# Nahuel-M/StereoVisionArray

Measured on NVIDIA B200. Metric: MDE/s, higher is better.
Workload: dtype u16

## Files before the change

stereovisionarray_b200/csrc/k_box.cu:

```cuda
#include <algorithm>

#include "sva_common.cuh"

#define BOX_THREADS 256
#define BOX_DP 16
#define BOX_CG 16
#define BOX_MAX_BAND 512

struct BoxParams {
    const uint16_t* A;
    void* out;
    int W, H, D, k, dmin, shift, cap;
    int gxp, gxn, gyp, gyn;
    int band_rows, txo;
    int apply_validity;
};

__device__ __forceinline__ int axis_limit(int pos, int dim, int k, int gp, int gn) {
    if (pos < k || pos >= dim - k) return -1;
    int lim = 0x7FFFFFFF;
    if (gp > 0) lim = min(lim, (pos - k) / gp);
    if (gn > 0) lim = min(lim, (dim - k - pos) / gn);
    return lim;
}

#define BOX_STAGES 3

__device__ __forceinline__ void box_cp16(uint32_t dst, const void* src, int src_bytes) {
    asm volatile("cp.async.cg.shared.global [%0], [%1], 16, %2;" ::"r"(dst), "l"(src), "r"(src_bytes) : "memory");
}

template <int NC, bool RAW>
__global__ void __launch_bounds__(BOX_THREADS, NC == 8 ? 3 : 4)
k_box_cost(BoxParams q) {
    constexpr int TXI = BOX_CG * NC;
    constexpr int ROW_BYTES = TXI * 64;
    constexpr int STAGE_BYTES = 2 * ROW_BYTES;
    extern __shared__ __align__(16) unsigned char box_smem[];
    unsigned char* s_ring = box_smem;
    uint2 (*s_P)[BOX_DP] = reinterpret_cast<uint2 (*)[BOX_DP]>(box_smem + BOX_STAGES * STAGE_BYTES);
    uint2 (*s_tot)[BOX_DP] = reinterpret_cast<uint2 (*)[BOX_DP]>(box_smem + BOX_STAGES * STAGE_BYTES + TXI * BOX_DP * 8);
    int* s_limy = reinterpret_cast<int*>(box_smem + BOX_STAGES * STAGE_BYTES + TXI * BOX_DP * 8 + BOX_CG * BOX_DP * 8);

    const int t = threadIdx.x, dp = t & (BOX_DP - 1), cg = t >> 4;
    const int W = q.W, H = q.H, D = q.D, k = q.k;
    const int d0 = blockIdx.y * 32;
    const int d = d0 + 2 * dp;
    const bool d_ok = d < D;
    const int xs = blockIdx.x * q.txo - k;
    const int y0 = blockIdx.z * q.band_rows, y1 = min(H, y0 + q.band_rows);
    if (y0 >= H) return;

    for (int i = t; i < y1 - y0; i += BOX_THREADS) s_limy[i] = q.apply_validity ? axis_limit(y0 + i, H, k, q.gyp, q.gyn) : 0x7FFFFFFF;

    int limx[NC];
    uint32_t v0[NC], v1[NC];
#pragma unroll
    for (int j = 0; j < NC; j++) {
        int x = xs + cg * NC + j;
        limx[j] = q.apply_validity ? axis_limit(x, W, k, q.gxp, q.gxn) : 0x7FFFFFFF;
        v0[j] = 0; v1[j] = 0;
    }
    const long long rowstride = (long long)W * D;
    const uint32_t ring_base = (uint32_t)__cvta_generic_to_shared(s_ring);

    auto fill = [&](int it) {
        const uint32_t st = ring_base + ((it + 2 * k) % BOX_STAGES) * STAGE_BYTES;
        const int ra = y0 + it + k - 1, rs = y0 + it - k;
        const bool ra_ok = ra >= 0 && ra < H, rs_ok = it >= 0 && rs >= 0 && rs < H;
#pragma unroll
        for (int c = t; c < TXI * 4; c += BOX_THREADS) {
            const int col = c >> 2, part = c & 3, x = xs + col, dd = d0 + 8 * part;
            const bool in = x >= 0 && x < W && dd < D;
            const long long off = ((long long)(in ? x : 0)) * D + (in ? dd : 0);
            box_cp16(st + c * 16, q.A + (ra_ok ? ra : 0) * rowstride + off, (in && ra_ok) ? 16 : 0);
            if (it >= 0) box_cp16(st + ROW_BYTES + c * 16, q.A + (rs_ok ? rs : 0) * rowstride + off, (in && rs_ok) ? 16 : 0);
        }
    };

    const int it_begin = -(2 * k - 1), it_end = y1 - y0;
#pragma unroll
    for (int i = 0; i < BOX_STAGES - 1; i++) {
        if (it_begin + i < it_end) fill(it_begin + i);
        asm volatile("cp.async.commit_group;" ::: "memory");
    }

    for (int it = it_begin; it < it_end; it++) {
        asm volatile("cp.async.wait_group %0;" ::"n"(BOX_STAGES - 2) : "memory");
        __syncthreads();
        if (it + BOX_STAGES - 1 < it_end) fill(it + BOX_STAGES - 1);
        asm volatile("cp.async.commit_group;" ::: "memory");
        const unsigned char* st = s_ring + ((it + 2 * k) % BOX_STAGES) * STAGE_BYTES;
        const uint32_t* rowa = reinterpret_cast<const uint32_t*>(st) + (cg * NC) * 16 + dp;
#pragma unroll
        for (int j = 0; j < NC; j++) { uint32_t w = rowa[j * 16]; v0[j] += w & 0xFFFFu; v1[j] += w >> 16; }
        if (it < 0) continue;
        const int y = y0 + it;
        uint32_t p0[NC], p1[NC];
        uint32_t a0 = 0, a1 = 0;
#pragma unroll
        for (int j = 0; j < NC; j++) { a0 += v0[j]; a1 += v1[j]; p0[j] = a0; p1[j] = a1; }
        s_tot[cg][dp] = make_uint2(a0, a1);
        __syncthreads();
        uint32_t o0 = 0, o1 = 0;
        for (int g = 0; g < cg; g++) { uint2 tt = s_tot[g][dp]; o0 += tt.x; o1 += tt.y; }
#pragma unroll
        for (int j = 0; j < NC; j++) s_P[cg * NC + j][dp] = make_uint2(p0[j] + o0, p1[j] + o1);
        __syncthreads();
        const int limy = s_limy[it];
#pragma unroll
        for (int j = 0; j < NC; j++) {
            int ci = cg * NC + j, x = xs + ci;
            if (ci < k || ci > TXI - k || x >= W || ci - k >= q.txo || !d_ok) continue;
            uint2 hi = s_P[ci + k - 1][dp];
            uint2 lo = (ci - k - 1 >= 0) ? s_P[ci - k - 1][dp] : make_uint2(0u, 0u);
            uint32_t r0 = hi.x - lo.x, r1 = hi.y - lo.y;
            int lim = min(limx[j], limy);
            bool ok0 = q.dmin + d <= lim, ok1 = q.dmin + d + 1 <= lim;
            long long o = ((long long)y * W + x) * D + d;
            if (RAW) {
                *reinterpret_cast<uint2*>((uint32_t*)q.out + o) = make_uint2(ok0 ? r0 : 0xFFFFFFFFu, ok1 ? r1 : 0xFFFFFFFFu);
            } else {
                uint32_t c0 = ok0 ? min((uint32_t)q.cap, r0 >> q.shift) : (uint32_t)q.cap;
                uint32_t c1 = ok1 ? min((uint32_t)q.cap, r1 >> q.shift) : (uint32_t)q.cap;
                *reinterpret_cast<uint32_t*>((uint16_t*)q.out + o) = c0 | (c1 << 16);
            }
        }
        const uint32_t* rows = reinterpret_cast<const uint32_t*>(st + ROW_BYTES) + (cg * NC) * 16 + dp;
#pragma unroll
        for (int j = 0; j < NC; j++) { uint32_t w = rows[j * 16]; v0[j] -= w & 0xFFFFu; v1[j] -= w >> 16; }
    }
}

template <int NC, bool RAW>
static cudaError_t box_launch(const BoxParams& q, dim3 grid, cudaStream_t stream) {
    constexpr int TXI = BOX_CG * NC;
    const size_t smem = (size_t)BOX_STAGES * 2 * TXI * 64 + (size_t)TXI * BOX_DP * 8 + BOX_CG * BOX_DP * 8 + BOX_MAX_BAND * 4;
    cudaError_t e = cudaFuncSetAttribute(k_box_cost<NC, RAW>, cudaFuncAttributeMaxDynamicSharedMemorySize, (int)smem);
    if (e != cudaSuccess) return e;
    k_box_cost<NC, RAW><<<grid, BOX_THREADS, smem, stream>>>(q);
    return cudaGetLastError();
}

int sva_launch_box(sva_ctx* ctx, const uint16_t* A, void* out, int W, int H, int D, int k, const sva_params* prm, bool raw, bool apply_validity) {
    if (k < 1 || k > 56) return ctx->fail(SVA_ERR_BAD_ARG, "win_half must be in 1..56");
    if (D % 8) return ctx->fail(SVA_ERR_BAD_ARG, "box filter needs a multiple of 8 planes");
    BoxParams q{};
    q.A = A; q.out = out; q.W = W; q.H = H; q.D = D; q.k = k;
    q.dmin = prm ? prm->min_disp : 0; q.shift = prm ? prm->cost_shift : 0; q.cap = prm ? prm->cost_cap : SVA_COST_CAP_MAX;
    q.apply_validity = apply_validity ? 1 : 0;
    if (prm && apply_validity) {
        for (int i = 0; i < prm->n_pairs; i++) {
            int gx = prm->pair_gx[i], gy = prm->pair_gy[i];
            if (gx > 0) q.gxp = gx > q.gxp ? gx : q.gxp;
            if (gx < 0) q.gxn = -gx > q.gxn ? -gx : q.gxn;
            if (gy > 0) q.gyp = gy > q.gyp ? gy : q.gyp;
            if (gy < 0) q.gyn = -gy > q.gyn ? -gy : q.gyn;
        }
    }
    const bool wide = k > 12;
    const int txi = wide ? 128 : 64;
    q.txo = txi - 2 * k + 1;
    int strips = div_up(W, q.txo), dch = div_up(D, 32);
    int bands = div_up(2 * ctx->sm_count * 2, strips * dch);
    int min_band = 4 * k > 32 ? 4 * k : 32;
    if (bands > H / min_band) bands = H / min_band;
    if (bands < 1) bands = 1;
    if (div_up(H, bands) > BOX_MAX_BAND) bands = div_up(H, BOX_MAX_BAND);
    q.band_rows = div_up(H, bands);
    bands = div_up(H, q.band_rows);
    dim3 grid(strips, dch, bands);
    LaunchScope ls(ctx, raw ? "k_box_cost_raw" : "k_box_cost");
    cudaError_t e;
    if (wide) e = raw ? box_launch<8, true>(q, grid, ctx->stream) : box_launch<8, false>(q, grid, ctx->stream);
    else e = raw ? box_launch<4, true>(q, grid, ctx->stream) : box_launch<4, false>(q, grid, ctx->stream);
    SVA_CUDA_OK(ctx, e);
    return SVA_OK;
}

#define BXP_WARPS 8
#define BXP_TCOLS 48
#define BXP_OPITCH 260
#define BXP_MAX_BAND 1024

struct BoxPParams {
    const uint32_t* AP;
    uint16_t* C;
    int W, H, D, k, kk, dmin, shift, cap;
    int gxp, gxn, gyp, gyn;
    int band_rows, txo, wp;
    int l2hint;
    int chunk;
    long long row_words;
    int ry0, ry1;
};

__global__ void __launch_bounds__(256, 2)
k_box_planar(BoxPParams q) {
    __shared__ __align__(16) uint32_t s_out[2][BXP_WARPS][BXP_OPITCH];
    __shared__ __align__(8) unsigned long long s_bar[2];
    __shared__ uint2 s_T[BXP_WARPS][8 * BXP_TCOLS];
    __shared__ int s_limy[BXP_MAX_BAND];
    const int t = threadIdx.x, lane = t & 31, warp = t >> 5;
    const int W = q.W, H = q.H, D = q.D, k = q.k;
    const int dpc = min((int)blockIdx.y * BXP_WARPS + warp, (D >> 1) - 1);
    const int d = 2 * dpc;
    const int xs = blockIdx.x * q.txo - q.kk;
    const int y0 = q.ry0 + blockIdx.z * q.band_rows, y1 = min(q.ry1, y0 + q.band_rows);
    for (int i = t; i < y1 - y0; i += 256) s_limy[i] = axis_limit(y0 + i, H, k, q.gyp, q.gyn);

    int thr[8], thrmin = 0x7FFFFFFF;
#pragma unroll
    for (int j = 0; j < 8; j++) {
        thr[j] = axis_limit(xs + lane * 8 + j, W, k, q.gxp, q.gxn) - q.dmin - d;
        thrmin = min(thrmin, thr[j]);
    }
    uint2* tbl = &s_T[warp][8 + lane];
    if (lane == 0) tbl[0] = make_uint2(0u, 0u);
    const uint32_t bar0 = (uint32_t)__cvta_generic_to_shared(&s_bar[0]);
    if (t == 0) {
        asm volatile("mbarrier.init.shared::cta.b64 [%0], %1;" ::"r"(bar0), "r"(BXP_WARPS) : "memory");
        asm volatile("mbarrier.init.shared::cta.b64 [%0], %1;" ::"r"(bar0 + 8), "r"(BXP_WARPS) : "memory");
    }
    int offh[8], offl[8];
#pragma unroll
    for (int j = 0; j < 8; j++) {
        offh[j] = ((j + k) & 7) * BXP_TCOLS + ((j + k) >> 3);
        offl[j] = ((j - k) & 7) * BXP_TCOLS + ((j - k) >> 3);
    }
    __syncthreads();

    const uint32_t* pz = q.AP + (size_t)dpc * q.wp + (size_t)blockIdx.x * q.txo + lane * 8;
    const uint32_t* pe = pz + (size_t)y0 * q.row_words;
    const long long back = 2LL * k * q.row_words;
    const int N = (y1 - y0) + 2 * k - 1;
    uint32_t F[8], Vh[8];
#pragma unroll
    for (int j = 0; j < 8; j++) { F[j] = 0; Vh[j] = 0; }

    const int hf = t & 1;
    const bool half_ok = (int)blockIdx.y * 16 + 8 * hf < D;
    const int xl0 = t >> 1, xl1 = xl0 + 128;
    const bool st0 = half_ok && xl0 >= q.kk && xl0 < q.kk + q.txo && xs + xl0 < W;
    const bool st1 = half_ok && xl1 >= q.kk && xl1 < q.kk + q.txo && xs + xl1 < W;
    uint16_t* po = q.C + ((size_t)y0 * W + (xs + xl0)) * D + blockIdx.y * 16 + 8 * hf;
    const size_t orow = (size_t)W * D;
    const uint32_t kB = (uint32_t)k << 16;

    auto store_row = [&](const int r) {
        const uint32_t bar = bar0 + 8 * (r & 1), parity = (uint32_t)(r >> 1) & 1u;
        asm volatile(
            "{\n"
            ".reg .pred p;\n"
            "BOXWAIT_%=:\n"
            "mbarrier.try_wait.parity.shared::cta.b64 p, [%0], %1;\n"
            "@p bra BOXDONE_%=;\n"
            "bra BOXWAIT_%=;\n"
            "BOXDONE_%=:\n"
            "}" ::"r"(bar), "r"(parity) : "memory");
        const uint32_t* src = &s_out[r & 1][4 * hf][xl0];
        if (st0) *reinterpret_cast<uint4*>(po) = make_uint4(src[0], src[BXP_OPITCH], src[2 * BXP_OPITCH], src[3 * BXP_OPITCH]);
        if (st1) *reinterpret_cast<uint4*>(po + 128 * D) = make_uint4(src[128], src[BXP_OPITCH + 128], src[2 * BXP_OPITCH + 128], src[3 * BXP_OPITCH + 128]);
        po += orow;
    };
    auto row = [&](const int n, const uint4& e0, const uint4& e1, const uint4& l0, const uint4& l1) {
        {
            const uint32_t ee[8] = {e0.x, e0.y, e0.z, e0.w, e1.x, e1.y, e1.z, e1.w};
            const uint32_t ll[8] = {l0.x, l0.y, l0.z, l0.w, l1.x, l1.y, l1.z, l1.w};
#pragma unroll
            for (int j = 0; j < 8; j++) {
                const uint32_t u = ee[j] - ll[j] + 0x80008000u;
                F[j] += u;
                Vh[j] += u >> 16;
            }
        }
        if (n < 2 * k - 1) return;
        const int it = n - (2 * k - 1);
        uint32_t pF[8], pV[8];
        pF[0] = F[0]; pV[0] = Vh[0];
#pragma unroll
        for (int j = 1; j < 8; j++) { pF[j] = pF[j - 1] + F[j]; pV[j] = pV[j - 1] + Vh[j]; }
        uint32_t incF = pF[7], incV = pV[7];
#pragma unroll
        for (int s = 1; s < 32; s <<= 1) {
            const uint32_t a = __shfl_up_sync(0xffffffffu, incF, s), b = __shfl_up_sync(0xffffffffu, incV, s);
            if (lane >= s) { incF += a; incV += b; }
        }
        const uint32_t exF = incF - pF[7], exV = incV - pV[7];
        __syncwarp();
#pragma unroll
        for (int j = 0; j < 8; j++)
            tbl[((j + 1) & 7) * BXP_TCOLS + ((j + 1) >> 3)] = make_uint2(pF[j] + exF, pV[j] + exV);
        __syncwarp();
        const uint32_t B = (uint32_t)(n + 1) * kB, B2 = B * 65537u;
        const int srow = s_limy[it] - q.dmin - d;
        uint32_t w[8];
        if (__all_sync(0xffffffffu, min(thrmin, srow) >= 1)) {
#pragma unroll
            for (int j = 0; j < 8; j++) {
                const uint2 hi = tbl[offh[j]], lo = tbl[offl[j]];
                const uint32_t chi = hi.y - lo.y - B;
                const uint32_t clo = hi.x - lo.x - B2 - (chi << 16);
                const uint32_t c0 = min(clo >> q.shift, (uint32_t)q.cap), c1 = min(chi >> q.shift, (uint32_t)q.cap);
                w[j] = c1 * 65536u + c0;
            }
        } else {
#pragma unroll
            for (int j = 0; j < 8; j++) {
                const uint2 hi = tbl[offh[j]], lo = tbl[offl[j]];
                const uint32_t chi = hi.y - lo.y - B;
                const uint32_t clo = hi.x - lo.x - B2 - (chi << 16);
                uint32_t c0 = min(clo >> q.shift, (uint32_t)q.cap), c1 = min(chi >> q.shift, (uint32_t)q.cap);
                const int m = min(thr[j], srow);
                c0 = m >= 0 ? c0 : (uint32_t)q.cap;
                c1 = m >= 1 ? c1 : (uint32_t)q.cap;
                w[j] = c1 * 65536u + c0;
            }
        }
        if (it > 0) store_row(it - 1);
        uint32_t* so = &s_out[it & 1][warp][lane * 8];
        *reinterpret_cast<uint4*>(so) = make_uint4(w[0], w[1], w[2], w[3]);
        *reinterpret_cast<uint4*>(so + 4) = make_uint4(w[4], w[5], w[6], w[7]);
        __syncwarp();
        if (lane == 0) asm volatile("mbarrier.arrive.shared::cta.b64 _, [%0];" ::"r"(bar0 + 8 * (it & 1)) : "memory");
    };

    uint4 a0 = ldg_stream_u128(pe), a1 = ldg_stream_u128(pe + 4), al0 = make_uint4(0, 0, 0, 0), al1 = al0;
    uint4 b0 = a0, b1 = a1, bl0 = al0, bl1 = al1;
    auto fetch = [&](const int n, uint4& e0, uint4& e1, uint4& l0, uint4& l1) {
        if (n < N) {
            pe += q.row_words;
            const uint32_t* pl = n >= 2 * k ? pe - back : pz;
            e0 = ldg_stream_u128(pe); e1 = ldg_stream_u128(pe + 4);
            l0 = ldg_stream_u128(pl); l1 = ldg_stream_u128(pl + 4);
        }
    };
    for (int n = 0; n < N; n += 2) {
        fetch(n + 1, b0, b1, bl0, bl1);
        row(n, a0, a1, al0, al1);
        if (n + 1 >= N) break;
        fetch(n + 2, a0, a1, al0, al1);
        row(n + 1, b0, b1, bl0, bl1);
    }
    store_row(y1 - y0 - 1);
}

template <int K, int PF, int OCC>
__global__ void __launch_bounds__(256, OCC)
k_box_planar_shfl(BoxPParams q) {
    static_assert(K % 8 == 4 && K >= 4 && K <= 56, "window half-width must be 4 mod 8");
    constexpr int M = (K - 4) / 8;
    __shared__ __align__(16) uint32_t s_out[2][BXP_WARPS][BXP_OPITCH];
    __shared__ __align__(8) unsigned long long s_bar[2];
    __shared__ int s_limy[BXP_MAX_BAND];
    const int t = threadIdx.x, lane = t & 31, warp = t >> 5;
    const int W = q.W, H = q.H, D = q.D;
    const int dpc = min((int)blockIdx.y * BXP_WARPS + warp, (D >> 1) - 1);
    const int d = 2 * dpc;
    const int xs = blockIdx.x * q.txo - K;
    const int y0 = q.ry0 + blockIdx.z * q.band_rows, y1 = min(q.ry1, y0 + q.band_rows);
    for (int i = t; i < y1 - y0; i += 256) s_limy[i] = axis_limit(y0 + i, H, K, q.gyp, q.gyn);

    int thr[8], thrmin = 0x7FFFFFFF;
#pragma unroll
    for (int j = 0; j < 8; j++) {
        thr[j] = axis_limit(xs + lane * 8 + j, W, K, q.gxp, q.gxn) - q.dmin - d;
        thrmin = min(thrmin, thr[j]);
    }
    const uint32_t bar0 = (uint32_t)__cvta_generic_to_shared(&s_bar[0]);
    if (t == 0) {
        asm volatile("mbarrier.init.shared::cta.b64 [%0], %1;" ::"r"(bar0), "r"(BXP_WARPS) : "memory");
        asm volatile("mbarrier.init.shared::cta.b64 [%0], %1;" ::"r"(bar0 + 8), "r"(BXP_WARPS) : "memory");
    }
    __syncthreads();

    const unsigned long long pol_enter = q.l2hint ? l2_policy_evict_last() : l2_policy_evict_normal();
    const unsigned long long pol_leave = q.l2hint ? l2_policy_evict_first() : l2_policy_evict_normal();
    const uint32_t* pe = q.AP + (size_t)dpc * q.wp + (size_t)blockIdx.x * q.txo + lane * 8 + (size_t)y0 * q.row_words;
    const long long back = 2LL * K * q.row_words;
    const int N = (y1 - y0) + 2 * K - 1;
    uint32_t F[8], Hh[8];
#pragma unroll
    for (int j = 0; j < 8; j++) { F[j] = 0; Hh[j] = 0; }

    const int hf = t & 1;
    const bool half_ok = (int)blockIdx.y * 16 + 8 * hf < D;
    const int xl0 = t >> 1, xl1 = xl0 + 128;
    const bool st0 = half_ok && xl0 >= K && xl0 < K + q.txo && xs + xl0 < W;
    const bool st1 = half_ok && xl1 >= K && xl1 < K + q.txo && xs + xl1 < W;
    uint16_t* po = q.C + ((size_t)y0 * W + (xs + xl0)) * D + blockIdx.y * 16 + 8 * hf;
    const size_t orow = (size_t)W * D;

    auto store_row = [&](const int r) {
        const uint32_t bar = bar0 + 8 * (r & 1), parity = (uint32_t)(r >> 1) & 1u;
        asm volatile(
            "{\n"
            ".reg .pred p;\n"
            "BOXSWAIT_%=:\n"
            "mbarrier.try_wait.parity.shared::cta.b64 p, [%0], %1;\n"
            "@p bra BOXSDONE_%=;\n"
            "bra BOXSWAIT_%=;\n"
            "BOXSDONE_%=:\n"
            "}" ::"r"(bar), "r"(parity) : "memory");
        const uint32_t* src = &s_out[r & 1][4 * hf][xl0];
        if (st0) stg_u128_hint(po, make_uint4(src[0], src[BXP_OPITCH], src[2 * BXP_OPITCH], src[3 * BXP_OPITCH]), pol_leave);
        if (st1) stg_u128_hint(po + 128 * D, make_uint4(src[128], src[BXP_OPITCH + 128], src[2 * BXP_OPITCH + 128], src[3 * BXP_OPITCH + 128]), pol_leave);
        po += orow;
    };
    auto hpass = [&](const uint32_t (&u)[8]) {
        uint32_t tF = ((u[0] + u[1]) + (u[2] + u[3])) + ((u[4] + u[5]) + (u[6] + u[7]));
        uint32_t tH = (((u[0] >> 16) + (u[1] >> 16)) + ((u[2] >> 16) + (u[3] >> 16))) + (((u[4] >> 16) + (u[5] >> 16)) + ((u[6] >> 16) + (u[7] >> 16)));
        uint32_t dF[8], dH[8];
        dF[4] = tF; dH[4] = tH;
#pragma unroll
        for (int s = 1; s <= M; s++) {
            dF[4] += __shfl_up_sync(0xffffffffu, tF, s) + __shfl_down_sync(0xffffffffu, tF, s);
            dH[4] += __shfl_up_sync(0xffffffffu, tH, s) + __shfl_down_sync(0xffffffffu, tH, s);
        }
#pragma unroll
        for (int i = 0; i < 3; i++) {
            const uint32_t hi = __shfl_down_sync(0xffffffffu, u[i], M + 1);
            const uint32_t lo = M == 0 ? u[i] : __shfl_up_sync(0xffffffffu, u[i], M == 0 ? 1 : M);
            dF[5 + i] = dF[4 + i] + hi - lo;
            dH[5 + i] = dH[4 + i] + (uint32_t)((int32_t)(hi - lo + 0x8000u) >> 16);
        }
#pragma unroll
        for (int i = 0; i < 4; i++) {
            const uint32_t hi = M == 0 ? u[7 - i] : __shfl_down_sync(0xffffffffu, u[7 - i], M == 0 ? 1 : M);
            const uint32_t lo = __shfl_up_sync(0xffffffffu, u[7 - i], M + 1);
            dF[3 - i] = dF[4 - i] - hi + lo;
            dH[3 - i] = dH[4 - i] - (uint32_t)((int32_t)(hi - lo + 0x8000u) >> 16);
        }
        constexpr uint32_t BF = (uint32_t)(2 * K) * 0x80008000u, BH = (uint32_t)(2 * K) * 0x8000u;
#pragma unroll
        for (int j = 0; j < 8; j++) { F[j] += dF[j] - BF; Hh[j] += dH[j] - BH; }
    };
    auto emit = [&](const int it) {
        const int srow = s_limy[it] - q.dmin - d;
        uint32_t w[8];
        if (__all_sync(0xffffffffu, min(thrmin, srow) >= 1)) {
#pragma unroll
            for (int j = 0; j < 8; j++) {
                const uint32_t chi = Hh[j], clo = F[j] - (chi << 16);
                const uint32_t c0 = min(clo >> q.shift, (uint32_t)q.cap), c1 = min(chi >> q.shift, (uint32_t)q.cap);
                w[j] = c1 * 65536u + c0;
            }
        } else {
#pragma unroll
            for (int j = 0; j < 8; j++) {
                const uint32_t chi = Hh[j], clo = F[j] - (chi << 16);
                uint32_t c0 = min(clo >> q.shift, (uint32_t)q.cap), c1 = min(chi >> q.shift, (uint32_t)q.cap);
                const int m = min(thr[j], srow);
                c0 = m >= 0 ? c0 : (uint32_t)q.cap;
                c1 = m >= 1 ? c1 : (uint32_t)q.cap;
                w[j] = c1 * 65536u + c0;
            }
        }
        if (it > 0) store_row(it - 1);
        uint32_t* so = &s_out[it & 1][warp][lane * 8];
        const bool swz = (lane & 4) != 0;
        *reinterpret_cast<uint4*>(so + (swz ? 4 : 0)) = swz ? make_uint4(w[4], w[5], w[6], w[7]) : make_uint4(w[0], w[1], w[2], w[3]);
        *reinterpret_cast<uint4*>(so + (swz ? 0 : 4)) = swz ? make_uint4(w[0], w[1], w[2], w[3]) : make_uint4(w[4], w[5], w[6], w[7]);
        __syncwarp();
        if (lane == 0) asm volatile("mbarrier.arrive.shared::cta.b64 _, [%0];" ::"r"(bar0 + 8 * (it & 1)) : "memory");
    };

    {
        uint32_t acc[8];
#pragma unroll
        for (int j = 0; j < 8; j++) acc[j] = 0x80008000u;
        int cnt = 0;
        U32x8 a = ldg_stream_u256(pe, pol_enter);
        for (int n = 0; n < 2 * K - 1; n++) {
            U32x8 b = a;
            if (n + 1 < 2 * K - 1) { pe += q.row_words; b = ldg_stream_u256(pe, pol_enter); }
#pragma unroll
            for (int j = 0; j < 8; j++) acc[j] += a.v[j];
            if (++cnt == q.chunk || n + 1 == 2 * K - 1) {
                hpass(acc);
#pragma unroll
                for (int j = 0; j < 8; j++) acc[j] = 0x80008000u;
                cnt = 0;
            }
            a = b;
        }
    }
    {
        const int R = y1 - y0;
        auto fetch = [&](const int it, U32x8& e, U32x8& l) {
            if (it < R) {
                pe += q.row_words;
                e = ldg_stream_u256(pe, pol_enter);
                if (it > 0) l = ldg_stream_u256(pe - back, pol_leave);
            }
        };
        auto row = [&](const int it, const U32x8& e, const U32x8& l) {
            uint32_t u[8];
#pragma unroll
            for (int j = 0; j < 8; j++) u[j] = e.v[j] - l.v[j] + 0x80008000u;
            hpass(u);
            emit(it);
        };
        U32x8 be[PF + 1], bl[PF + 1];
#pragma unroll
        for (int i = 0; i <= PF; i++)
#pragma unroll
            for (int j = 0; j < 8; j++) { be[i].v[j] = 0; bl[i].v[j] = 0; }
#pragma unroll
        for (int i = 0; i < PF; i++) fetch(i, be[i], bl[i]);
        for (int it = 0; it < R; it += PF + 1) {
#pragma unroll
            for (int i = 0; i <= PF; i++) {
                if (it + i < R) {
                    fetch(it + i + PF, be[(i + PF) % (PF + 1)], bl[(i + PF) % (PF + 1)]);
                    row(it + i, be[i], bl[i]);
                }
            }
        }
        store_row(R - 1);
    }
    (void)N;
}

int sva_ap_prepare(sva_ctx* ctx);
int sva_ap_unpack(sva_ctx* ctx);

static int sva_launch_box_planar(sva_ctx* ctx) {
    const sva_params& p = ctx->prm;
    const int W = p.width, H = p.height, D = p.num_disp, k = p.win_half;
    BoxPParams q{};
    q.AP = ctx->AP.as<uint32_t>(); q.C = ctx->C.as<uint16_t>();
    q.W = W; q.H = H; q.D = D; q.k = k; q.kk = ctx->ap.padl; q.dmin = p.min_disp; q.shift = p.cost_shift; q.cap = p.cost_cap;
    for (int i = 0; i < p.n_pairs; i++) {
        int gx = p.pair_gx[i], gy = p.pair_gy[i];
        if (gx > 0) q.gxp = gx > q.gxp ? gx : q.gxp;
        if (gx < 0) q.gxn = -gx > q.gxn ? -gx : q.gxn;
        if (gy > 0) q.gyp = gy > q.gyp ? gy : q.gyp;
        if (gy < 0) q.gyn = -gy > q.gyn ? -gy : q.gyn;
    }
    q.txo = ctx->ap.txo; q.wp = ctx->ap.wp; q.row_words = (long long)ctx->ap.row_words;
    const int strips = ctx->ap.strips, dgroups = div_up(D, 16);
    const bool shfl = ctx->tune_box_shfl && k % 8 == 4;
    auto shfl_kernel = [&](int occ) -> void (*)(BoxPParams) {
        switch (k) {
            case 4: return occ == 3 ? k_box_planar_shfl<4, 1, 3> : k_box_planar_shfl<4, 1, 2>;
            case 12: return occ == 3 ? k_box_planar_shfl<12, 1, 3> : k_box_planar_shfl<12, 1, 2>;
            case 20: return occ == 3 ? k_box_planar_shfl<20, 1, 3> : k_box_planar_shfl<20, 1, 2>;
            case 28: return occ == 3 ? k_box_planar_shfl<28, 1, 3> : k_box_planar_shfl<28, 1, 2>;
            case 36: return occ == 3 ? k_box_planar_shfl<36, 1, 3> : k_box_planar_shfl<36, 1, 2>;
            case 44: return occ == 3 ? k_box_planar_shfl<44, 1, 3> : k_box_planar_shfl<44, 1, 2>;
            default: return occ == 3 ? k_box_planar_shfl<52, 1, 3> : k_box_planar_shfl<52, 1, 2>;
        }
    };
    if (shfl) {
        q.chunk = std::max(1, 32767 / (255 * p.n_pairs));
        q.l2hint = ctx->tune_box_l2 ? 1 : 0;
    }
    q.ry0 = 0; q.ry1 = H;
    if (ctx->win_rows > 0) { q.ry0 = ctx->win_y0; q.ry1 = ctx->win_y0 + ctx->win_rows; }
    const int Hw = q.ry1 - q.ry0;
    void (*kern)(BoxPParams) = k_box_planar;
    const char* label = shfl ? "k_box_planar_shfl" : "k_box_planar";
    int bands = 1;
    double best = 1e30;
    const int per_band = strips * dgroups;
    for (int occ = 2; occ <= (shfl ? 3 : 2); occ++) {
        if (shfl && ctx->tune_box_occ && occ != ctx->tune_box_occ) continue;
        void (*cand)(BoxPParams) = shfl ? shfl_kernel(occ) : k_box_planar;
        int per_sm = occ;
        SVA_CUDA_OK(ctx, cudaOccupancyMaxActiveBlocksPerMultiprocessor(&per_sm, cand, 256, 0));
        if (per_sm < 1) per_sm = 1;
        const int slots = per_sm * ctx->sm_count;
        const double warm = shfl ? (2 * k - 1) / 3.0 + div_up(2 * k - 1, q.chunk) : (double)(2 * k - 1);
        for (int b = 1; b <= Hw && b <= 4096; b++) {
            const int rows = div_up(Hw, b);
            if (rows > BXP_MAX_BAND) continue;
            if (b > 1 && rows < k) break;
            const int nb = div_up(Hw, rows);
            const double cost = (double)div_up(nb * per_band, slots) * per_sm * (rows + warm + 8);
            if (cost < best) { best = cost; bands = nb; q.band_rows = rows; kern = cand; }
        }
    }
    if (ctx->tune_box_bands > 0) {
        const int rows = std::min(BXP_MAX_BAND, std::max(1, div_up(Hw, ctx->tune_box_bands)));
        q.band_rows = rows; bands = div_up(Hw, rows);
    }
    LaunchScope ls(ctx, label);
    kern<<<dim3(strips, dgroups, bands), 256, 0, ctx->stream>>>(q);
    SVA_CUDA_OK(ctx, cudaGetLastError());
    return SVA_OK;
}

int sva_run_box(sva_ctx* ctx, bool raw) {
    const sva_params& p = ctx->prm;
    size_t cells = (size_t)p.width * p.height * p.num_disp;
    if (raw) {
        SVA_TRY(ctx->reserve(ctx->Craw, cells * sizeof(uint32_t)));
        SVA_TRY(sva_ap_unpack(ctx));
        return sva_launch_box(ctx, ctx->A.as<uint16_t>(), ctx->Craw.p, p.width, p.height, p.num_disp, p.win_half, &p, true, true);
    }
    SVA_TRY(ctx->reserve(ctx->C, cells * sizeof(uint16_t)));
    SVA_TRY(sva_launch_box_planar(ctx));
    ctx->have_cost = true;
    return SVA_OK;
}
```

Measured before the change: 129,400.

## Cache sliding-window leaving rows in tensor memory instead of reloading from global

When the kernel runs at two CTAs per SM, each CTA allocates 256 columns of Blackwell tensor memory. Each warp stores incoming rows of the vertical box window into a ring of TMEM slots. The leaving row is then read back from TMEM rather than re-fetched from global/L2, which is meant to cut the second global load per output row. The cost is tcgen05 alloc/dealloc plus extra fences, barriers and synchronous TMEM load/store waits. Only part of the window fits (at most 16 rows), so the remaining rows still come from global memory.

```diff
diff --git a/stereovisionarray_b200/csrc/k_box.cu b/stereovisionarray_b200/csrc/k_box.cu
--- a/stereovisionarray_b200/csrc/k_box.cu
+++ b/stereovisionarray_b200/csrc/k_box.cu
@@ -345,14 +345,28 @@
     store_row(y1 - y0 - 1);
 }
 
+__device__ __forceinline__ void tmem_st8(const uint32_t taddr, const uint32_t (&v)[8]) {
+    asm volatile("tcgen05.st.sync.aligned.32x32b.x8.b32 [%0], {%1, %2, %3, %4, %5, %6, %7, %8};"
+                 ::"r"(taddr), "r"(v[0]), "r"(v[1]), "r"(v[2]), "r"(v[3]), "r"(v[4]), "r"(v[5]), "r"(v[6]), "r"(v[7]) : "memory");
+}
+__device__ __forceinline__ void tmem_ld8(const uint32_t taddr, uint32_t (&v)[8]) {
+    asm volatile("tcgen05.wait::st.sync.aligned;\n"
+                 "tcgen05.ld.sync.aligned.32x32b.x8.b32 {%0, %1, %2, %3, %4, %5, %6, %7}, [%8];\n"
+                 "tcgen05.wait::ld.sync.aligned;"
+                 : "=r"(v[0]), "=r"(v[1]), "=r"(v[2]), "=r"(v[3]), "=r"(v[4]), "=r"(v[5]), "=r"(v[6]), "=r"(v[7]) : "r"(taddr) : "memory");
+}
 template <int K, int PF, int OCC>
 __global__ void __launch_bounds__(256, OCC)
 k_box_planar_shfl(BoxPParams q) {
     static_assert(K % 8 == 4 && K >= 4 && K <= 56, "window half-width must be 4 mod 8");
+    static_assert(OCC == 2 || OCC == 3, "tensor memory is split for 2 CTAs per SM");
     constexpr int M = (K - 4) / 8;
+    constexpr int TM_COLS = OCC == 2 ? 256 : 0;
+    constexpr int TM_ROWS = 2 * K < TM_COLS / 16 ? 2 * K : TM_COLS / 16;
     __shared__ __align__(16) uint32_t s_out[2][BXP_WARPS][BXP_OPITCH];
     __shared__ __align__(8) unsigned long long s_bar[2];
     __shared__ int s_limy[BXP_MAX_BAND];
+    __shared__ uint32_t s_tmem;
     const int t = threadIdx.x, lane = t & 31, warp = t >> 5;
     const int W = q.W, H = q.H, D = q.D;
     const int dpc = min((int)blockIdx.y * BXP_WARPS + warp, (D >> 1) - 1);
@@ -372,7 +386,14 @@
         asm volatile("mbarrier.init.shared::cta.b64 [%0], %1;" ::"r"(bar0), "r"(BXP_WARPS) : "memory");
         asm volatile("mbarrier.init.shared::cta.b64 [%0], %1;" ::"r"(bar0 + 8), "r"(BXP_WARPS) : "memory");
     }
+    if (TM_COLS > 0 && warp == 0) {
+        asm volatile("tcgen05.alloc.cta_group::1.sync.aligned.shared::cta.b32 [%0], %1;" ::"r"((uint32_t)__cvta_generic_to_shared(&s_tmem)), "n"(TM_COLS) : "memory");
+        asm volatile("tcgen05.relinquish_alloc_permit.cta_group::1.sync.aligned;" ::: "memory");
+    }
+    if (TM_COLS > 0) asm volatile("tcgen05.fence::before_thread_sync;" ::: "memory");
     __syncthreads();
+    if (TM_COLS > 0) asm volatile("tcgen05.fence::after_thread_sync;" ::: "memory");
+    const uint32_t tm_warp = TM_COLS == 0 ? 0u : s_tmem + ((uint32_t)(warp & 3) << 21) + (uint32_t)(warp >> 2) * (TM_COLS / 2);
 
     const unsigned long long pol_enter = q.l2hint ? l2_policy_evict_last() : l2_policy_evict_normal();
     const unsigned long long pol_leave = q.l2hint ? l2_policy_evict_first() : l2_policy_evict_normal();
@@ -474,6 +495,7 @@
         for (int n = 0; n < 2 * K - 1; n++) {
             U32x8 b = a;
             if (n + 1 < 2 * K - 1) { pe += q.row_words; b = ldg_stream_u256(pe, pol_enter); }
+            if (n < TM_ROWS) tmem_st8(tm_warp + 8 * n, a.v);
 #pragma unroll
             for (int j = 0; j < 8; j++) acc[j] += a.v[j];
             if (++cnt == q.chunk || n + 1 == 2 * K - 1) {
@@ -487,17 +509,26 @@
     }
     {
         const int R = y1 - y0;
+        int fslot = 2 * K - 1, slot = 2 * K - 1;
         auto fetch = [&](const int it, U32x8& e, U32x8& l) {
             if (it < R) {
                 pe += q.row_words;
                 e = ldg_stream_u256(pe, pol_enter);
-                if (it > 0) l = ldg_stream_u256(pe - back, pol_leave);
+                if (it > 0 && fslot >= TM_ROWS) l = ldg_stream_u256(pe - back, pol_leave);
+                fslot = fslot + 1 == 2 * K ? 0 : fslot + 1;
             }
         };
         auto row = [&](const int it, const U32x8& e, const U32x8& l) {
-            uint32_t u[8];
-#pragma unroll
-            for (int j = 0; j < 8; j++) u[j] = e.v[j] - l.v[j] + 0x80008000u;
+            uint32_t lv[8], u[8];
+#pragma unroll
+            for (int j = 0; j < 8; j++) lv[j] = l.v[j];
+            if (slot < TM_ROWS) {
+                if (it > 0) tmem_ld8(tm_warp + 8 * slot, lv);
+                tmem_st8(tm_warp + 8 * slot, e.v);
+            }
+            slot = slot + 1 == 2 * K ? 0 : slot + 1;
+#pragma unroll
+            for (int j = 0; j < 8; j++) u[j] = e.v[j] - lv[j] + 0x80008000u;
             hpass(u);
             emit(it);
         };
@@ -520,6 +551,12 @@
         store_row(R - 1);
     }
     (void)N;
+    if (TM_COLS > 0) asm volatile("tcgen05.fence::before_thread_sync;" ::: "memory");
+    if (TM_COLS > 0) __syncthreads();
+    if (TM_COLS > 0 && warp == 0) {
+        asm volatile("tcgen05.fence::after_thread_sync;" ::: "memory");
+        asm volatile("tcgen05.dealloc.cta_group::1.sync.aligned.b32 %0, %1;" ::"r"(s_tmem), "n"(TM_COLS) : "memory");
+    }
 }
 
 int sva_ap_prepare(sva_ctx* ctx);
```

New measurement: 118,900 (median of 6 runs). -8.1%, worse.
